# Hi-FT/ERD

Hardware: AMD Instinct MI355X
Metric: images/sec GFL-R50 40+40 incre step @1333x800 (higher is better)
Workload: dtype f32; 1 GPU; gfl_r50_fpn first_40_incre_last_40 ERD (BASELINE configs[1]), 1333x800 padded to 800x1344, fp32, procedural weights; batch_per_gpu=4, global_batch=4, parallelism=dp1

## Files before the change

### erd_amd/csrc/erd_common.h

```cpp
#pragma once
#include <hip/hip_runtime.h>
#include <stdint.h>
#include <stdio.h>
#include <stdarg.h>
#include "../../include/erd_hip.h"
#include "erd_probes.h"

namespace erd {

void set_error(const char* fmt, ...);
int usable_cus(int physical);

bool conv_thin_x3_ok(const erd_conv_desc* d);
int conv_thin_x3(const erd_conv_desc* d, hipStream_t st);
bool conv_thin_bf16_ok(const erd_conv_desc* d);
int conv_thin_bf16(const erd_conv_desc* d, hipStream_t st);

inline int check_launch(const char* what) {
    hipError_t e = hipGetLastError();
    if (e != hipSuccess) {
        set_error("%s: %s", what, hipGetErrorString(e));
        return (int)e;
    }
    return 0;
}

#define ERD_REQUIRE(cond, ...)            \
    do {                                  \
        if (!(cond)) {                    \
            erd::set_error(__VA_ARGS__);  \
            return ERD_EINVAL;            \
        }                                 \
    } while (0)

#define ERD_ZERO_ASYNC(p, bytes, st)                                           \
    do {                                                                       \
        const hipError_t e_ = hipMemsetAsync((p), 0, (bytes), (st));           \
        if (e_ != hipSuccess) {                                                \
            erd::set_error("hipMemsetAsync: %s", hipGetErrorString(e_));       \
            return (int)e_;                                                    \
        }                                                                      \
    } while (0)

__device__ __forceinline__ float wave_sum(float v) {
#pragma unroll
    for (int o = 32; o > 0; o >>= 1) v += __shfl_xor(v, o, 64);
    return v;
}
__device__ __forceinline__ float wave_sum_dpp(float v) {
#define ERD_DPP_ADD(ctrl) v += __builtin_bit_cast(float, __builtin_amdgcn_update_dpp(0, __builtin_bit_cast(int, v), ctrl, 0xF, 0xF, true))
    ERD_DPP_ADD(0xB1);
    ERD_DPP_ADD(0x4E);
    ERD_DPP_ADD(0x141);
    ERD_DPP_ADD(0x140);
#undef ERD_DPP_ADD
    const int b = __builtin_bit_cast(int, v);
    return (__builtin_bit_cast(float, __builtin_amdgcn_readlane(b, 0)) + __builtin_bit_cast(float, __builtin_amdgcn_readlane(b, 16))) +
           (__builtin_bit_cast(float, __builtin_amdgcn_readlane(b, 32)) + __builtin_bit_cast(float, __builtin_amdgcn_readlane(b, 48)));
}
__device__ __forceinline__ double wave_sum_d(double v) {
#pragma unroll
    for (int o = 32; o > 0; o >>= 1) v += __shfl_xor(v, o, 64);
    return v;
}
__device__ __forceinline__ float wave_max(float v) {
#pragma unroll
    for (int o = 32; o > 0; o >>= 1) v = fmaxf(v, __shfl_xor(v, o, 64));
    return v;
}

typedef __bf16 bf16x2_t __attribute__((ext_vector_type(2)));
typedef float f32x2_t __attribute__((ext_vector_type(2)));
__device__ __forceinline__ unsigned pack2_bf16(float a, float b) {
    const f32x2_t v = {a, b};
    return __builtin_bit_cast(unsigned, __builtin_convertvector(v, bf16x2_t));
}
__device__ __forceinline__ float bf16_lo(unsigned u) { return __uint_as_float(u << 16); }
__device__ __forceinline__ float bf16_hi(unsigned u) { return __uint_as_float(u & 0xffff0000u); }
__device__ __forceinline__ float4 unpack4_bf16(uint2 u) {
    return make_float4(bf16_lo(u.x), bf16_hi(u.x), bf16_lo(u.y), bf16_hi(u.y));
}
__device__ __forceinline__ uint2 pack4_bf16(float4 v) { return make_uint2(pack2_bf16(v.x, v.y), pack2_bf16(v.z, v.w)); }

template <typename T>
__device__ __forceinline__ T* uniform_ptr(T* p) {
    const unsigned long long v = reinterpret_cast<unsigned long long>(p);
    const unsigned lo = __builtin_amdgcn_readfirstlane((unsigned)v), hi = __builtin_amdgcn_readfirstlane((unsigned)(v >> 32));
    return reinterpret_cast<T*>(((unsigned long long)hi << 32) | lo);
}
__device__ __forceinline__ int uniform_int(int v) { return __builtin_amdgcn_readfirstlane(v); }

__device__ __forceinline__ int xcd_contiguous(unsigned block, int grid) {
    const int q = grid >> 3, r = grid & 7, xcd = block & 7, idx = block >> 3;
    return (xcd < r ? xcd * (q + 1) : r * (q + 1) + (xcd - r) * q) + idx;
}

__device__ __forceinline__ float scalar_op(float v) {
    asm("" : "+v"(v));
    return v;
}
__device__ __forceinline__ void limbs3_pair(float x0, float x1, unsigned& hi, unsigned& mid, unsigned& lo) {
    hi = pack2_bf16(x0, x1);
    const float r0 = scalar_op(x0 - bf16_lo(hi)), r1 = scalar_op(x1 - bf16_hi(hi));
    mid = pack2_bf16(r0, r1);
    lo = pack2_bf16(scalar_op(r0 - bf16_lo(mid)), scalar_op(r1 - bf16_hi(mid)));
}
__device__ __forceinline__ void limbs3(float x, unsigned short& hi, unsigned short& mid, unsigned short& lo) {
    unsigned h, m, l;
    limbs3_pair(x, 0.f, h, m, l);
    hi = (unsigned short)(h & 0xffffu);
    mid = (unsigned short)(m & 0xffffu);
    lo = (unsigned short)(l & 0xffffu);
}

__device__ __forceinline__ void wino_x3_weight_item(const float* __restrict__ w, unsigned short* __restrict__ U3, int Cout, int Cin,
                                                    int flip, int co, int ci) {
    float g[3][3];
#pragma unroll
    for (int a = 0; a < 3; ++a)
#pragma unroll
        for (int b = 0; b < 3; ++b)
            g[a][b] = co < Cout ? w[((int64_t)co * 9 + (flip ? 8 - (a * 3 + b) : a * 3 + b)) * Cin + ci] : 0.f;
    float t[4][3];
#pragma unroll
    for (int b = 0; b < 3; ++b) {
        t[0][b] = g[0][b];
        t[1][b] = 0.5f * (g[0][b] + g[1][b] + g[2][b]);
        t[2][b] = 0.5f * (g[0][b] - g[1][b] + g[2][b]);
        t[3][b] = g[2][b];
    }
    const int nks = Cin / 16, ncb32 = (Cout + 31) / 32;
    const int64_t per_xl = (int64_t)ncb32 * nks * 512;
    const int64_t base = (((int64_t)(co / 32) * nks + ci / 16) * 64 + ((ci % 16) / 8) * 32 + (co % 32)) * 8 + (ci % 8);
#pragma unroll
    for (int i = 0; i < 4; ++i) {
        const float u[4] = {t[i][0], 0.5f * (t[i][0] + t[i][1] + t[i][2]), 0.5f * (t[i][0] - t[i][1] + t[i][2]), t[i][2]};
#pragma unroll
        for (int j = 0; j < 4; ++j) {
            unsigned short hi, mid, lo;
            limbs3(u[j], hi, mid, lo);
            const int64_t o = (int64_t)((i * 4 + j) * 3) * per_xl + base;
            U3[o] = hi;
            U3[o + per_xl] = mid;
            U3[o + 2 * per_xl] = lo;
        }
    }
}

struct bf16s { unsigned short bits; };
__device__ __forceinline__ float4 ld4(const float* p) { return *reinterpret_cast<const float4*>(p); }
__device__ __forceinline__ float4 ld4(const bf16s* p) { return unpack4_bf16(*reinterpret_cast<const uint2*>(p)); }
__device__ __forceinline__ void st4(float* p, float4 v) { *reinterpret_cast<float4*>(p) = v; }
__device__ __forceinline__ void st4(bf16s* p, float4 v) { *reinterpret_cast<uint2*>(p) = pack4_bf16(v); }
__device__ __forceinline__ float ld1(const float* p) { return *p; }
__device__ __forceinline__ float ld1(const bf16s* p) { return __uint_as_float((unsigned)p->bits << 16); }
__device__ __forceinline__ void st1(float* p, float v) { *p = v; }
__device__ __forceinline__ void st1(bf16s* p, float v) { p->bits = (unsigned short)(pack2_bf16(v, 0.f) & 0xffffu); }

}
```

### erd_amd/csrc/prep.hip

```cpp
#include "erd_common.h"

namespace {

__device__ __forceinline__ void transpose_block(const erd_weight_prep_item& it, int local, float (*tile)[33]) {
    const int nbx = (it.Cin + 31) / 32, nby = (it.Cout + 31) / 32;
    const int bx = local % nbx, by = (local / nbx) % nby, t = local / (nbx * nby);
    const int td = it.flip ? it.ntaps - 1 - t : t;
    const int ci0 = bx * 32, co0 = by * 32;
    const int tx = threadIdx.x & 31, ty = threadIdx.x >> 5;
    const float* __restrict__ w = it.w;
    for (int r = ty; r < 32; r += 8) {
        const int co = co0 + r, ci = ci0 + tx;
        float v = 0.f;
        if (co < it.Cout && ci < it.Cin) v = w[((int64_t)co * it.ntaps + t) * it.Cin + ci] * (it.rowscale ? it.rowscale[co] : 1.f);
        tile[r][tx] = v;
    }
    __syncthreads();
    for (int r = ty; r < 32; r += 8) {
        const int ci = ci0 + r, co = co0 + tx;
        if (co < it.Cout && ci < it.Cin) {
            const int64_t o = ((int64_t)ci * it.ntaps + td) * it.Cout + co;
            if (it.kind == 1) reinterpret_cast<__bf16*>(it.dst)[o] = (__bf16)tile[tx][r];
            else reinterpret_cast<float*>(it.dst)[o] = tile[tx][r];
        }
    }
}

__device__ __forceinline__ void wino_block(const erd_weight_prep_item& it, int local) {
    const int Cout = it.Cout, Cin = it.Cin, flip = it.flip;
    const float* __restrict__ w = it.w;
    float* __restrict__ U = reinterpret_cast<float*>(it.dst);
    const int cop = (Cout + 15) / 16 * 16;
    const int64_t idx = local * 256ll + threadIdx.x;
    if (idx >= (int64_t)cop * Cin) return;
    const int co = (int)(idx / Cin), ci = (int)(idx % Cin);
    float g[3][3];
#pragma unroll
    for (int a = 0; a < 3; ++a)
#pragma unroll
        for (int b = 0; b < 3; ++b)
            g[a][b] = co < Cout ? w[((int64_t)co * 9 + (flip ? 8 - (a * 3 + b) : a * 3 + b)) * Cin + ci] : 0.f;
    float t[4][3];
#pragma unroll
    for (int b = 0; b < 3; ++b) {
        t[0][b] = g[0][b];
        t[1][b] = 0.5f * (g[0][b] + g[1][b] + g[2][b]);
        t[2][b] = 0.5f * (g[0][b] - g[1][b] + g[2][b]);
        t[3][b] = g[2][b];
    }
    const int nks = Cin / 16;
    const int64_t per_xi = (int64_t)(cop / 16) * nks * 256;
    const int64_t base = (((int64_t)(co / 16) * nks + ci / 16) * 4 + (ci % 16) / 4) * 64 + (co % 16) * 4 + (ci % 4);
#pragma unroll
    for (int i = 0; i < 4; ++i) {
        const float u0 = t[i][0], u1 = 0.5f * (t[i][0] + t[i][1] + t[i][2]), u2 = 0.5f * (t[i][0] - t[i][1] + t[i][2]),
                    u3 = t[i][2];
        U[(i * 4 + 0) * per_xi + base] = u0;
        U[(i * 4 + 1) * per_xi + base] = u1;
        U[(i * 4 + 2) * per_xi + base] = u2;
        U[(i * 4 + 3) * per_xi + base] = u3;
    }
}

__device__ __forceinline__ void split3_block(const erd_weight_prep_item& it, int local) {
    const int64_t n = (int64_t)it.Cout * it.ntaps * it.Cin;
    const int64_t i = local * 256ll + threadIdx.x;
    if (i >= n) return;
    unsigned short h, m, l;
    erd::limbs3(it.w[i], h, m, l);
    unsigned short* d = reinterpret_cast<unsigned short*>(it.dst);
    d[i] = h;
    d[n + i] = m;
    d[2 * n + i] = l;
}

__device__ __forceinline__ void wino_x3_block(const erd_weight_prep_item& it, int local) {
    const int cop = (it.Cout + 31) / 32 * 32;
    const int64_t idx = local * 256ll + threadIdx.x;
    if (idx >= (int64_t)cop * it.Cin) return;
    erd::wino_x3_weight_item(it.w, reinterpret_cast<unsigned short*>(it.dst), it.Cout, it.Cin, it.flip, (int)(idx / it.Cin), (int)(idx % it.Cin));
}

__global__ __launch_bounds__(256) void weight_prep_kernel(const erd_weight_prep_item* __restrict__ items, int nitems) {
    __shared__ float tile[32][33];
    __shared__ int s_item;
    if (threadIdx.x == 0) {
        int lo = 0, hi = nitems - 1;
        while (lo < hi) {
            const int mid = (lo + hi + 1) >> 1;
            if (items[mid].block0 <= (int)blockIdx.x) lo = mid; else hi = mid - 1;
        }
        s_item = lo;
    }
    __syncthreads();
    const erd_weight_prep_item it = items[s_item];
    const int local = (int)blockIdx.x - it.block0;
    if (it.kind == 2) wino_block(it, local);
    else if (it.kind == 3) split3_block(it, local);
    else if (it.kind == 4) wino_x3_block(it, local);
    else transpose_block(it, local, tile);
}

}

extern "C" int erd_weight_prep_blocks(int kind, int Cout, int ntaps, int Cin) {
    if (kind == 2) return (int)(((int64_t)((Cout + 15) / 16 * 16) * Cin + 255) / 256);
    if (kind == 3) return (int)(((int64_t)Cout * ntaps * Cin + 255) / 256);
    if (kind == 4) return (int)(((int64_t)((Cout + 31) / 32 * 32) * Cin + 255) / 256);
    return ((Cin + 31) / 32) * ((Cout + 31) / 32) * ntaps;
}

extern "C" int erd_weight_prep_batch(const erd_weight_prep_item* items_dev, int nitems, int total_blocks, erd_stream_t stream) {
    ERD_REQUIRE(items_dev && nitems >= 0 && total_blocks >= 0, "weight_prep_batch: bad args");
    if (nitems == 0 || total_blocks == 0) return 0;
    hipLaunchKernelGGL(weight_prep_kernel, dim3((unsigned)total_blocks), dim3(256), 0, (hipStream_t)stream, items_dev, nitems);
    return erd::check_launch("weight_prep_batch");
}
```

Before: 124.3 images/sec.

## Vectorize weight prep kernels and use persistent grid over work units

Rewrites the batched weight-preparation kernel so each workgroup processes a contiguous range of work units with a grid capped at a few workgroups per CU, instead of one block per unit with a binary search each. Transpose tiles grow to 64x64 with float4 loads and vectorized bf16 and f32 stores. Winograd and x3-limb Winograd transforms now handle vectors of input channels per thread, and the limb split uses 4-wide loads and packed stores. The goal is to cut per-block overhead and scalar memory traffic in the per-step weight transforms, at the cost of more registers and more complex tail and alignment handling.

```diff
diff --git a/erd_amd/csrc/erd_common.h b/erd_amd/csrc/erd_common.h
--- a/erd_amd/csrc/erd_common.h
+++ b/erd_amd/csrc/erd_common.h
@@ -113,6 +113,10 @@
     lo = (unsigned short)(l & 0xffffu);
 }
 
+__device__ __forceinline__ float wino_g_row(int i, float g0, float g1, float g2) {
+    return i == 0 ? g0 : i == 1 ? 0.5f * (g0 + g1 + g2) : i == 2 ? 0.5f * (g0 - g1 + g2) : g2;
+}
+
 __device__ __forceinline__ void wino_x3_weight_item(const float* __restrict__ w, unsigned short* __restrict__ U3, int Cout, int Cin,
                                                     int flip, int co, int ci) {
     float g[3][3];
@@ -123,22 +127,18 @@
             g[a][b] = co < Cout ? w[((int64_t)co * 9 + (flip ? 8 - (a * 3 + b) : a * 3 + b)) * Cin + ci] : 0.f;
     float t[4][3];
 #pragma unroll
-    for (int b = 0; b < 3; ++b) {
-        t[0][b] = g[0][b];
-        t[1][b] = 0.5f * (g[0][b] + g[1][b] + g[2][b]);
-        t[2][b] = 0.5f * (g[0][b] - g[1][b] + g[2][b]);
-        t[3][b] = g[2][b];
-    }
+    for (int i = 0; i < 4; ++i)
+#pragma unroll
+        for (int b = 0; b < 3; ++b) t[i][b] = wino_g_row(i, g[0][b], g[1][b], g[2][b]);
     const int nks = Cin / 16, ncb32 = (Cout + 31) / 32;
     const int64_t per_xl = (int64_t)ncb32 * nks * 512;
     const int64_t base = (((int64_t)(co / 32) * nks + ci / 16) * 64 + ((ci % 16) / 8) * 32 + (co % 32)) * 8 + (ci % 8);
 #pragma unroll
     for (int i = 0; i < 4; ++i) {
-        const float u[4] = {t[i][0], 0.5f * (t[i][0] + t[i][1] + t[i][2]), 0.5f * (t[i][0] - t[i][1] + t[i][2]), t[i][2]};
 #pragma unroll
         for (int j = 0; j < 4; ++j) {
             unsigned short hi, mid, lo;
-            limbs3(u[j], hi, mid, lo);
+            limbs3(wino_g_row(j, t[i][0], t[i][1], t[i][2]), hi, mid, lo);
             const int64_t o = (int64_t)((i * 4 + j) * 3) * per_xl + base;
             U3[o] = hi;
             U3[o + per_xl] = mid;
diff --git a/erd_amd/csrc/prep.hip b/erd_amd/csrc/prep.hip
--- a/erd_amd/csrc/prep.hip
+++ b/erd_amd/csrc/prep.hip
@@ -1,118 +1,278 @@
 #include "erd_common.h"
+#include <algorithm>
 
 namespace {
 
-__device__ __forceinline__ void transpose_block(const erd_weight_prep_item& it, int local, float (*tile)[33]) {
-    const int nbx = (it.Cin + 31) / 32, nby = (it.Cout + 31) / 32;
+constexpr int TT = 64;
+constexpr int SPLIT_UNIT = 4096;
+constexpr int PREP_WGS_PER_CU = 8;
+
+__device__ __forceinline__ bool aligned16(const void* p) { return (reinterpret_cast<uintptr_t>(p) & 15) == 0; }
+
+#define ERD_GLOBAL __attribute__((address_space(1)))
+typedef float f32x4_t __attribute__((ext_vector_type(4)));
+typedef unsigned u32x4_t __attribute__((ext_vector_type(4)));
+typedef unsigned u32x2_t __attribute__((ext_vector_type(2)));
+__device__ __forceinline__ float gld1(const float* p) { return *(const ERD_GLOBAL float*)p; }
+__device__ __forceinline__ float4 gld4(const float* p) {
+    const f32x4_t v = *(const ERD_GLOBAL f32x4_t*)p;
+    return make_float4(v.x, v.y, v.z, v.w);
+}
+__device__ __forceinline__ void gst1(float* p, float v) { *(ERD_GLOBAL float*)p = v; }
+__device__ __forceinline__ void gst1(unsigned short* p, unsigned short v) { *(ERD_GLOBAL unsigned short*)p = v; }
+__device__ __forceinline__ void gst4(float* p, float4 v) { *(ERD_GLOBAL f32x4_t*)p = f32x4_t{v.x, v.y, v.z, v.w}; }
+__device__ __forceinline__ void gst8h(unsigned short* p, unsigned a, unsigned b, unsigned c, unsigned d) {
+    *(ERD_GLOBAL u32x4_t*)p = u32x4_t{a, b, c, d};
+}
+__device__ __forceinline__ void gst4h(unsigned short* p, unsigned a, unsigned b) { *(ERD_GLOBAL u32x2_t*)p = u32x2_t{a, b}; }
+__device__ __forceinline__ unsigned short bf16_bits(float v) { return (unsigned short)(erd::pack2_bf16(v, 0.f) & 0xffffu); }
+
+__device__ __forceinline__ void transpose_unit(const erd_weight_prep_item& it, int local, float (*tile)[TT + 1]) {
+    const int Cout = it.Cout, Cin = it.Cin, ntaps = it.ntaps;
+    const int nbx = (Cin + TT - 1) / TT, nby = (Cout + TT - 1) / TT;
     const int bx = local % nbx, by = (local / nbx) % nby, t = local / (nbx * nby);
-    const int td = it.flip ? it.ntaps - 1 - t : t;
-    const int ci0 = bx * 32, co0 = by * 32;
-    const int tx = threadIdx.x & 31, ty = threadIdx.x >> 5;
-    const float* __restrict__ w = it.w;
-    for (int r = ty; r < 32; r += 8) {
-        const int co = co0 + r, ci = ci0 + tx;
-        float v = 0.f;
-        if (co < it.Cout && ci < it.Cin) v = w[((int64_t)co * it.ntaps + t) * it.Cin + ci] * (it.rowscale ? it.rowscale[co] : 1.f);
-        tile[r][tx] = v;
+    const int td = it.flip ? ntaps - 1 - t : t;
+    const int ci0 = bx * TT, co0 = by * TT;
+    const float* __restrict__ w = it.w;
+    const float* __restrict__ rowscale = it.rowscale;
+    {
+        const bool vec = Cin % 4 == 0 && aligned16(w);
+        const int c = (threadIdx.x & 15) * 4, r0 = threadIdx.x >> 4;
+        float4 v[4];
+        float rs[4];
+#pragma unroll
+        for (int k = 0; k < 4; ++k) {
+            const int co = co0 + r0 + 16 * k, ci = ci0 + c;
+            v[k] = make_float4(0.f, 0.f, 0.f, 0.f);
+            rs[k] = 1.f;
+            if (co < Cout && ci < Cin) {
+                const float* p = w + ((int64_t)co * ntaps + t) * Cin + ci;
+                if (rowscale) rs[k] = gld1(rowscale + co);
+                if (vec) {
+                    v[k] = gld4(p);
+                } else {
+                    v[k].x = gld1(p);
+                    if (ci + 1 < Cin) v[k].y = gld1(p + 1);
+                    if (ci + 2 < Cin) v[k].z = gld1(p + 2);
+                    if (ci + 3 < Cin) v[k].w = gld1(p + 3);
+                }
+            }
+        }
+#pragma unroll
+        for (int k = 0; k < 4; ++k) {
+            float* row = tile[r0 + 16 * k] + c;
+            row[0] = v[k].x * rs[k];
+            row[1] = v[k].y * rs[k];
+            row[2] = v[k].z * rs[k];
+            row[3] = v[k].w * rs[k];
+        }
     }
     __syncthreads();
-    for (int r = ty; r < 32; r += 8) {
-        const int ci = ci0 + r, co = co0 + tx;
-        if (co < it.Cout && ci < it.Cin) {
-            const int64_t o = ((int64_t)ci * it.ntaps + td) * it.Cout + co;
-            if (it.kind == 1) reinterpret_cast<__bf16*>(it.dst)[o] = (__bf16)tile[tx][r];
-            else reinterpret_cast<float*>(it.dst)[o] = tile[tx][r];
-        }
-    }
-}
-
-__device__ __forceinline__ void wino_block(const erd_weight_prep_item& it, int local) {
+    if (it.kind == 1) {
+        unsigned short* __restrict__ d = reinterpret_cast<unsigned short*>(it.dst);
+        const bool vec = Cout % 8 == 0 && aligned16(d);
+        const int c = (threadIdx.x & 7) * 8;
+#pragma unroll
+        for (int k = 0; k < 2; ++k) {
+            const int r = (threadIdx.x >> 3) + 32 * k;
+            const int ci = ci0 + r, co = co0 + c;
+            if (ci >= Cin || co >= Cout) continue;
+            const int64_t o = ((int64_t)ci * ntaps + td) * Cout + co;
+            if (vec) {
+                gst8h(d + o, erd::pack2_bf16(tile[c][r], tile[c + 1][r]), erd::pack2_bf16(tile[c + 2][r], tile[c + 3][r]),
+                      erd::pack2_bf16(tile[c + 4][r], tile[c + 5][r]), erd::pack2_bf16(tile[c + 6][r], tile[c + 7][r]));
+            } else {
+#pragma unroll
+                for (int e = 0; e < 8; ++e)
+                    if (co + e < Cout) gst1(d + o + e, bf16_bits(tile[c + e][r]));
+            }
+        }
+    } else {
+        float* __restrict__ d = reinterpret_cast<float*>(it.dst);
+        const bool vec = Cout % 4 == 0 && aligned16(d);
+        const int c = (threadIdx.x & 15) * 4;
+#pragma unroll
+        for (int k = 0; k < 4; ++k) {
+            const int r = (threadIdx.x >> 4) + 16 * k;
+            const int ci = ci0 + r, co = co0 + c;
+            if (ci >= Cin || co >= Cout) continue;
+            const int64_t o = ((int64_t)ci * ntaps + td) * Cout + co;
+            if (vec) {
+                gst4(d + o, make_float4(tile[c][r], tile[c + 1][r], tile[c + 2][r], tile[c + 3][r]));
+            } else {
+#pragma unroll
+                for (int e = 0; e < 4; ++e)
+                    if (co + e < Cout) gst1(d + o + e, tile[c + e][r]);
+            }
+        }
+    }
+    __syncthreads();
+}
+
+__device__ __forceinline__ void wino_unit(const erd_weight_prep_item& it, int local) {
     const int Cout = it.Cout, Cin = it.Cin, flip = it.flip;
-    const float* __restrict__ w = it.w;
+    const int nks = Cin / 16, ngr = (nks + 3) / 4;
+    const int cb = local / ngr, s = (local % ngr) * 4 + (threadIdx.x >> 6);
+    if (s >= nks) return;
+    const int lane = threadIdx.x & 63, q = lane >> 4, co = cb * 16 + (lane & 15), ci = s * 16 + q * 4;
+    const float* __restrict__ w = it.w;
+    float4 g[9];
+#pragma unroll
+    for (int tap = 0; tap < 9; ++tap) {
+        g[tap] = gld4(w + ((int64_t)min(co, Cout - 1) * 9 + (flip ? 8 - tap : tap)) * Cin + ci);
+        if (co >= Cout) g[tap] = make_float4(0.f, 0.f, 0.f, 0.f);
+    }
     float* __restrict__ U = reinterpret_cast<float*>(it.dst);
-    const int cop = (Cout + 15) / 16 * 16;
-    const int64_t idx = local * 256ll + threadIdx.x;
-    if (idx >= (int64_t)cop * Cin) return;
-    const int co = (int)(idx / Cin), ci = (int)(idx % Cin);
-    float g[3][3];
-#pragma unroll
-    for (int a = 0; a < 3; ++a)
+    const int64_t per_xi = (int64_t)((Cout + 15) / 16) * nks * 256;
+    const int64_t base = (((int64_t)cb * nks + s) * 4 + q) * 64 + (lane & 15) * 4;
+#pragma unroll
+    for (int i = 0; i < 4; ++i) {
+        float4 t[3];
 #pragma unroll
         for (int b = 0; b < 3; ++b)
-            g[a][b] = co < Cout ? w[((int64_t)co * 9 + (flip ? 8 - (a * 3 + b) : a * 3 + b)) * Cin + ci] : 0.f;
-    float t[4][3];
-#pragma unroll
-    for (int b = 0; b < 3; ++b) {
-        t[0][b] = g[0][b];
-        t[1][b] = 0.5f * (g[0][b] + g[1][b] + g[2][b]);
-        t[2][b] = 0.5f * (g[0][b] - g[1][b] + g[2][b]);
-        t[3][b] = g[2][b];
-    }
-    const int nks = Cin / 16;
-    const int64_t per_xi = (int64_t)(cop / 16) * nks * 256;
-    const int64_t base = (((int64_t)(co / 16) * nks + ci / 16) * 4 + (ci % 16) / 4) * 64 + (co % 16) * 4 + (ci % 4);
+            t[b] = make_float4(erd::wino_g_row(i, g[b].x, g[3 + b].x, g[6 + b].x), erd::wino_g_row(i, g[b].y, g[3 + b].y, g[6 + b].y),
+                               erd::wino_g_row(i, g[b].z, g[3 + b].z, g[6 + b].z), erd::wino_g_row(i, g[b].w, g[3 + b].w, g[6 + b].w));
+#pragma unroll
+        for (int j = 0; j < 4; ++j)
+            gst4(U + (i * 4 + j) * per_xi + base,
+                     make_float4(erd::wino_g_row(j, t[0].x, t[1].x, t[2].x), erd::wino_g_row(j, t[0].y, t[1].y, t[2].y),
+                                 erd::wino_g_row(j, t[0].z, t[1].z, t[2].z), erd::wino_g_row(j, t[0].w, t[1].w, t[2].w)));
+    }
+}
+
+__device__ __forceinline__ void st4_limbs(unsigned short* p, unsigned a, unsigned b) {
+    if ((reinterpret_cast<uintptr_t>(p) & 7) == 0) {
+        gst4h(p, a, b);
+    } else {
+        gst1(p, (unsigned short)(a & 0xffffu));
+        gst1(p + 1, (unsigned short)(a >> 16));
+        gst1(p + 2, (unsigned short)(b & 0xffffu));
+        gst1(p + 3, (unsigned short)(b >> 16));
+    }
+}
+
+__device__ __forceinline__ void split3_unit(const erd_weight_prep_item& it, int local) {
+    const int64_t n = (int64_t)it.Cout * it.ntaps * it.Cin;
+    const float* __restrict__ w = it.w;
+    unsigned short* __restrict__ d = reinterpret_cast<unsigned short*>(it.dst);
+    const int head = (int)std::min<int64_t>(n, (int64_t)(((0 - reinterpret_cast<uintptr_t>(w)) >> 2) & 3));
+    const int64_t ngroups = (n - head) >> 2;
+    const int64_t g0 = (int64_t)local * (SPLIT_UNIT / 4) + threadIdx.x;
+    float4 v[4];
+#pragma unroll
+    for (int k = 0; k < 4; ++k)
+        if (g0 + 256 * k < ngroups) v[k] = gld4(w + head + 4 * (g0 + 256 * k));
+#pragma unroll
+    for (int k = 0; k < 4; ++k) {
+        if (g0 + 256 * k >= ngroups) continue;
+        const int64_t i = head + 4 * (g0 + 256 * k);
+        unsigned h0, m0, l0, h1, m1, l1;
+        erd::limbs3_pair(v[k].x, v[k].y, h0, m0, l0);
+        erd::limbs3_pair(v[k].z, v[k].w, h1, m1, l1);
+        st4_limbs(d + i, h0, h1);
+        st4_limbs(d + n + i, m0, m1);
+        st4_limbs(d + 2 * n + i, l0, l1);
+    }
+    if (local == 0 && (int64_t)threadIdx.x < n - 4 * ngroups) {
+        const int64_t i = (int)threadIdx.x < head ? (int64_t)threadIdx.x : 4 * ngroups + threadIdx.x;
+        unsigned short h, m, l;
+        erd::limbs3(gld1(w + i), h, m, l);
+        gst1(d + i, h);
+        gst1(d + n + i, m);
+        gst1(d + 2 * n + i, l);
+    }
+}
+
+__device__ __forceinline__ void wino_x3_unit(const erd_weight_prep_item& it, int local) {
+    const int Cout = it.Cout, Cin = it.Cin, flip = it.flip;
+    const int nks = Cin / 16, ngr = (nks + 3) / 4;
+    const int cb = local / ngr, s = (local % ngr) * 4 + (threadIdx.x >> 6);
+    if (s >= nks) return;
+    const int lane = threadIdx.x & 63, co = cb * 32 + (lane & 31), ci = s * 16 + (lane >> 5) * 8;
+    const float* __restrict__ w = it.w;
+    float g[9][8];
+#pragma unroll
+    for (int tap = 0; tap < 9; ++tap) {
+        const float* p = w + ((int64_t)min(co, Cout - 1) * 9 + (flip ? 8 - tap : tap)) * Cin + ci;
+        float4 a = gld4(p), b = gld4(p + 4);
+        if (co >= Cout) a = b = make_float4(0.f, 0.f, 0.f, 0.f);
+        g[tap][0] = a.x; g[tap][1] = a.y; g[tap][2] = a.z; g[tap][3] = a.w;
+        g[tap][4] = b.x; g[tap][5] = b.y; g[tap][6] = b.z; g[tap][7] = b.w;
+    }
+    unsigned short* __restrict__ U3 = reinterpret_cast<unsigned short*>(it.dst);
+    const int64_t per_xl = (int64_t)((Cout + 31) / 32) * nks * 512;
+    const int64_t base = (((int64_t)cb * nks + s) * 64 + lane) * 8;
 #pragma unroll
     for (int i = 0; i < 4; ++i) {
-        const float u0 = t[i][0], u1 = 0.5f * (t[i][0] + t[i][1] + t[i][2]), u2 = 0.5f * (t[i][0] - t[i][1] + t[i][2]),
-                    u3 = t[i][2];
-        U[(i * 4 + 0) * per_xi + base] = u0;
-        U[(i * 4 + 1) * per_xi + base] = u1;
-        U[(i * 4 + 2) * per_xi + base] = u2;
-        U[(i * 4 + 3) * per_xi + base] = u3;
-    }
-}
-
-__device__ __forceinline__ void split3_block(const erd_weight_prep_item& it, int local) {
-    const int64_t n = (int64_t)it.Cout * it.ntaps * it.Cin;
-    const int64_t i = local * 256ll + threadIdx.x;
-    if (i >= n) return;
-    unsigned short h, m, l;
-    erd::limbs3(it.w[i], h, m, l);
-    unsigned short* d = reinterpret_cast<unsigned short*>(it.dst);
-    d[i] = h;
-    d[n + i] = m;
-    d[2 * n + i] = l;
-}
-
-__device__ __forceinline__ void wino_x3_block(const erd_weight_prep_item& it, int local) {
-    const int cop = (it.Cout + 31) / 32 * 32;
-    const int64_t idx = local * 256ll + threadIdx.x;
-    if (idx >= (int64_t)cop * it.Cin) return;
-    erd::wino_x3_weight_item(it.w, reinterpret_cast<unsigned short*>(it.dst), it.Cout, it.Cin, it.flip, (int)(idx / it.Cin), (int)(idx % it.Cin));
-}
-
-__global__ __launch_bounds__(256) void weight_prep_kernel(const erd_weight_prep_item* __restrict__ items, int nitems) {
-    __shared__ float tile[32][33];
-    __shared__ int s_item;
-    if (threadIdx.x == 0) {
-        int lo = 0, hi = nitems - 1;
-        while (lo < hi) {
-            const int mid = (lo + hi + 1) >> 1;
-            if (items[mid].block0 <= (int)blockIdx.x) lo = mid; else hi = mid - 1;
-        }
-        s_item = lo;
-    }
-    __syncthreads();
-    const erd_weight_prep_item it = items[s_item];
-    const int local = (int)blockIdx.x - it.block0;
-    if (it.kind == 2) wino_block(it, local);
-    else if (it.kind == 3) split3_block(it, local);
-    else if (it.kind == 4) wino_x3_block(it, local);
-    else transpose_block(it, local, tile);
+        float t[3][8];
+#pragma unroll
+        for (int b = 0; b < 3; ++b)
+#pragma unroll
+            for (int e = 0; e < 8; ++e) t[b][e] = erd::wino_g_row(i, g[b][e], g[3 + b][e], g[6 + b][e]);
+#pragma unroll
+        for (int j = 0; j < 4; ++j) {
+            unsigned hi[4], mid[4], lo[4];
+#pragma unroll
+            for (int e = 0; e < 4; ++e)
+                erd::limbs3_pair(erd::wino_g_row(j, t[0][2 * e], t[1][2 * e], t[2][2 * e]),
+                                 erd::wino_g_row(j, t[0][2 * e + 1], t[1][2 * e + 1], t[2][2 * e + 1]), hi[e], mid[e], lo[e]);
+            unsigned short* o = U3 + (int64_t)((i * 4 + j) * 3) * per_xl + base;
+            gst8h(o, hi[0], hi[1], hi[2], hi[3]);
+            gst8h(o + per_xl, mid[0], mid[1], mid[2], mid[3]);
+            gst8h(o + 2 * per_xl, lo[0], lo[1], lo[2], lo[3]);
+        }
+    }
+}
+
+__global__ __launch_bounds__(256) void weight_prep_kernel(const erd_weight_prep_item* __restrict__ items, int nitems, int total) {
+    __shared__ float tile[TT][TT + 1];
+    const int b = (int)blockIdx.x, per = total / (int)gridDim.x, rem = total % (int)gridDim.x;
+    const int u0 = b * per + min(b, rem), u1 = u0 + per + (b < rem ? 1 : 0);
+    if (u0 >= u1) return;
+    int idx = 0;
+    for (int hi = nitems - 1; idx < hi;) {
+        const int mid = (idx + hi + 1) >> 1;
+        if (items[mid].block0 <= u0) idx = mid; else hi = mid - 1;
+    }
+    erd_weight_prep_item it = items[idx];
+    int next0 = idx + 1 < nitems ? items[idx + 1].block0 : total;
+    for (int u = u0; u < u1; ++u) {
+        while (u >= next0) {
+            it = items[++idx];
+            next0 = idx + 1 < nitems ? items[idx + 1].block0 : total;
+        }
+        const int local = u - it.block0;
+        if (it.kind == 2) wino_unit(it, local);
+        else if (it.kind == 3) split3_unit(it, local);
+        else if (it.kind == 4) wino_x3_unit(it, local);
+        else transpose_unit(it, local, tile);
+    }
+}
+
+int num_cus_prep() {
+    static int n = 0;
+    if (n == 0) {
+        int dev = 0;
+        hipDeviceProp_t prop;
+        if (hipGetDevice(&dev) == hipSuccess && hipGetDeviceProperties(&prop, dev) == hipSuccess) n = prop.multiProcessorCount;
+        if (n <= 0) n = 256;
+    }
+    return n;
 }
 
 }
 
 extern "C" int erd_weight_prep_blocks(int kind, int Cout, int ntaps, int Cin) {
-    if (kind == 2) return (int)(((int64_t)((Cout + 15) / 16 * 16) * Cin + 255) / 256);
-    if (kind == 3) return (int)(((int64_t)Cout * ntaps * Cin + 255) / 256);
-    if (kind == 4) return (int)(((int64_t)((Cout + 31) / 32 * 32) * Cin + 255) / 256);
-    return ((Cin + 31) / 32) * ((Cout + 31) / 32) * ntaps;
+    if (kind == 2) return ((Cout + 15) / 16) * ((Cin / 16 + 3) / 4);
+    if (kind == 3) return (int)(((int64_t)Cout * ntaps * Cin + SPLIT_UNIT - 1) / SPLIT_UNIT);
+    if (kind == 4) return ((Cout + 31) / 32) * ((Cin / 16 + 3) / 4);
+    return ((Cin + TT - 1) / TT) * ((Cout + TT - 1) / TT) * ntaps;
 }
 
 extern "C" int erd_weight_prep_batch(const erd_weight_prep_item* items_dev, int nitems, int total_blocks, erd_stream_t stream) {
     ERD_REQUIRE(items_dev && nitems >= 0 && total_blocks >= 0, "weight_prep_batch: bad args");
     if (nitems == 0 || total_blocks == 0) return 0;
-    hipLaunchKernelGGL(weight_prep_kernel, dim3((unsigned)total_blocks), dim3(256), 0, (hipStream_t)stream, items_dev, nitems);
+    const int grid = std::min(total_blocks, PREP_WGS_PER_CU * erd::usable_cus(num_cus_prep()));
+    hipLaunchKernelGGL(weight_prep_kernel, dim3((unsigned)grid), dim3(256), 0, (hipStream_t)stream, items_dev, nitems, total_blocks);
     return erd::check_launch("weight_prep_batch");
 }
```

New measurement: 124.8 images/sec, median of 6. No clear change (+0.4%).
